# ubc-vision/quadraturefields

Measured on AMD Instinct MI355X. Metric: rays/sec at 800x800 Lego (mesh-quadrature render: ray/mesh intersection + hash-grid/MLP field + compositing), higher is better.
Workload: dtype f32; 1 GPU; Lego 800x800 (configs[1]), 1xMI355X per frame, fp32 hash-grid + tiny-MLP HIP kernels; rays_per_frame=640000, max_hits=25, triangles=983040, log2_hashmap_size=19, up_sample=1, bvh_fallback_frames=0, overflow_repaired_frames=8, reorigin_rule_redone_frames=0, camera_mismatch_frames=0, frames_in_flight=1

## Files before the change

### quadraturefields_amd/csrc/raster.hip

```cpp
#include <type_traits>

#include "exact_common.h"

#pragma clang fp contract(off)

namespace {

struct RasterCam {
    float r00, r01, r02, r10, r11, r12, r20, r21, r22;
    float cx, cy, cz;
    float fx, fy, px0, py0;
    int w, h;
};

constexpr float kRasterGuard = 0.25f;

struct SlabArgs {
    float t_lo, t_hi;
    int stop_at;
    uint64_t *keys;
    const float4 *ray_rec;
};

struct TriSetup {
    int x0, x1, y0, y1;
    bool use_edges;
    float ea[3], eb[3], ec[3];
};

__device__ __forceinline__ bool tri_setup(const float4 a, const float4 b, const float4 c, const RasterCam &cam, TriSetup &s)
{
    float minx = INFINITY, maxx = -INFINITY, miny = INFINITY, maxy = -INFINITY;
    int behind = 0;
    const float4 vs[3] = {a, b, c};
    float sxs[3], sys[3];
#pragma unroll
    for (int k = 0; k < 3; ++k) {
        const float dx = vs[k].x - cam.cx, dy = vs[k].y - cam.cy, dz = vs[k].z - cam.cz;
        const float xc = cam.r00 * dx + cam.r10 * dy + cam.r20 * dz;
        const float yc = cam.r01 * dx + cam.r11 * dy + cam.r21 * dz;
        const float zc = cam.r02 * dx + cam.r12 * dy + cam.r22 * dz;
        const float zv = -zc;
        if (!(zv > 1e-6f)) { ++behind; sxs[k] = sys[k] = 0.0f; continue; }
        const float sx = cam.fx * (xc / zv) + cam.px0;
        const float sy = -cam.fy * (yc / zv) + cam.py0;
        sxs[k] = sx; sys[k] = sy;
        minx = fminf(minx, sx); maxx = fmaxf(maxx, sx);
        miny = fminf(miny, sy); maxy = fmaxf(maxy, sy);
    }
    if (behind == 3) return false;
    s.use_edges = false;
    if (behind > 0) {
        s.x0 = 0; s.y0 = 0; s.x1 = cam.w - 1; s.y1 = cam.h - 1;
    } else {
        s.x0 = (int)fmaxf(floorf(minx - kRasterGuard), 0.0f);
        s.y0 = (int)fmaxf(floorf(miny - kRasterGuard), 0.0f);
        s.x1 = (int)fminf(ceilf(maxx + kRasterGuard), (float)(cam.w - 1));
        s.y1 = (int)fminf(ceilf(maxy + kRasterGuard), (float)(cam.h - 1));
        if (!(maxx + kRasterGuard >= 0.0f) || !(maxy + kRasterGuard >= 0.0f) ||
            !(minx - kRasterGuard <= (float)(cam.w - 1)) || !(miny - kRasterGuard <= (float)(cam.h - 1)))
            return false;
        const float area2 = (sxs[1] - sxs[0]) * (sys[2] - sys[0]) - (sys[1] - sys[0]) * (sxs[2] - sxs[0]);
        if (fabsf(area2) > 1e-2f) {
            s.use_edges = true;
            const float sgn = area2 > 0.0f ? 1.0f : -1.0f;
#pragma unroll
            for (int k = 0; k < 3; ++k) {
                const int k1 = (k + 1) % 3;
                const float ex = sxs[k1] - sxs[k], ey = sys[k1] - sys[k];
                s.ea[k] = -sgn * ey;
                s.eb[k] = sgn * ex;
                s.ec[k] = -(s.ea[k] * sxs[k] + s.eb[k] * sys[k]) + (kRasterGuard + 0.05f) * (fabsf(ex) + fabsf(ey)) + 1e-3f;
            }
        }
    }
    return true;
}

constexpr int kBinStage = 256;
constexpr int kBinIdBits = 26;
struct BinStage { int n; int tile[kBinStage]; uint2 rec[kBinStage]; };
struct TileBins {
    int32_t *cursor;
    uint2 *bins;
    int cap;
    BinStage *stage;
};

__device__ __forceinline__ void bin_records(const TileBins &tb, int tile, uint2 rec)
{
    const int lane = (int)__lane_id();
    for (;;) {
        const int t0 = __builtin_amdgcn_readfirstlane(tile);
        const unsigned long long m = __ballot(tile == t0);
        if (tile == t0) {
            const int rank = __popcll(m & ((1ull << lane) - 1ull));
            int base = 0;
            if (rank == 0) base = atomicAdd(&tb.cursor[t0], __popcll(m));
            base = __shfl(base, __ffsll((long long)m) - 1, 64);
            if (base + rank < tb.cap) tb.bins[(int64_t)t0 * tb.cap + base + rank] = rec;
            break;
        }
    }
}

template <int kRasterLanes, bool kWide, bool kSlab = false, bool kBins = false>
__device__ __forceinline__ void raster_triangle(const float4 *__restrict__ tris, int64_t tri_i, int sub, const RasterCam &cam,
                                                const float *__restrict__ rays_o, const float *__restrict__ rays_d,
                                                int max_hits, int32_t *__restrict__ hit_tri, float *__restrict__ hit_t,
                                                int32_t *__restrict__ hit_count, int32_t *__restrict__ overflow,
                                                const bool cam_origin, const SlabArgs slab = SlabArgs(),
                                                const TileBins bins = TileBins())
{
    const float4 a = tris[tri_i * 3 + 0], b = tris[tri_i * 3 + 1], c = tris[tri_i * 3 + 2];
    const int id = __float_as_int(a.w);
    TriSetup ts;
    if (!tri_setup(a, b, c, cam, ts)) return;
    const int x0 = ts.x0, x1 = ts.x1, y0 = ts.y0, y1 = ts.y1;
    const bool use_edges = ts.use_edges;
    const float *ea = ts.ea, *eb = ts.eb, *ec = ts.ec;
    const int bw = x1 - x0 + 1;
    const int total = bw * (y1 - y0 + 1);
    int px = x0 + sub % bw, py = y0 + sub / bw;
    for (int q = sub; q < total; q += kRasterLanes) {
        const int cx_ = px, cy_ = py;
        px += kRasterLanes;
        while (px > x1) { px -= bw; ++py; }
        if (use_edges) {
            const float fx_ = (float)cx_, fy_ = (float)cy_;
            if (ea[0] * fx_ + eb[0] * fy_ + ec[0] < 0.0f || ea[1] * fx_ + eb[1] * fy_ + ec[1] < 0.0f ||
                ea[2] * fx_ + eb[2] * fy_ + ec[2] < 0.0f)
                continue;
        }
        const int64_t ray = (int64_t)cy_ * cam.w + cx_;
        float dx, dy, dz;
        if (kSlab && slab.ray_rec) {
            const float4 rr = slab.ray_rec[ray];
            if (__float_as_int(rr.w) >= slab.stop_at) continue;
            dx = rr.x; dy = rr.y; dz = rr.z;
        } else {
            dx = rays_d[ray * 3]; dy = rays_d[ray * 3 + 1]; dz = rays_d[ray * 3 + 2];
        }
        float ox = cam.cx, oy = cam.cy, oz = cam.cz;
        if (!cam_origin) { ox = rays_o[ray * 3]; oy = rays_o[ray * 3 + 1]; oz = rays_o[ray * 3 + 2]; }
        asm volatile("" : "+v"(ox), "+v"(oy), "+v"(oz), "+v"(dx), "+v"(dy), "+v"(dz));
        float t;
        if (!mt_hit(a, b, c, ox, oy, oz, dx, dy, dz, &t)) continue;
        if (kSlab) {
            if (!(t >= slab.t_lo && t < slab.t_hi)) continue;
            const int slot = atomicAdd(&hit_count[ray], 1);
            if (slot < max_hits) slab.keys[(int64_t)slot * ((int64_t)cam.w * cam.h) + ray] = hit_key(t, id);
            else atomicAdd(overflow, 1);
            continue;
        }
        if (kBins) {
            const int tile = (cy_ >> 3) * ((cam.w + 7) >> 3) + (cx_ >> 3);
            const uint2 rec = make_uint2(__float_as_uint(t), ((uint32_t)id << 6) | (uint32_t)((cy_ & 7) * 8 + (cx_ & 7)));
            const int at = atomicAdd(&bins.stage->n, 1);
            if (at < kBinStage) { bins.stage->tile[at] = tile; bins.stage->rec[at] = rec; }
            else bin_records(bins, tile, rec);
            continue;
        }
        const int slot = atomicAdd(&hit_count[ray], 1);
        if (slot < max_hits) {
            const int64_t at = kWide ? (int64_t)slot * ((int64_t)cam.w * cam.h) + ray : ray * max_hits + slot;
            hit_t[at] = t;
            if (hit_tri) hit_tri[at] = id;
        } else {
            atomicAdd(overflow, 1);
        }
    }
}

template <int kRasterLanes, bool kWide>
__global__ __launch_bounds__(256) void raster_kernel(const float4 *__restrict__ tris, int64_t n_tri, RasterCam cam,
                                                     const float *__restrict__ rays_o, const float *__restrict__ rays_d,
                                                     int max_hits, int32_t *__restrict__ hit_tri, float *__restrict__ hit_t,
                                                     int32_t *__restrict__ hit_count, int32_t *__restrict__ overflow,
                                                     const int32_t *__restrict__ ray_flag)
{
    const int64_t gid = (int64_t)blockIdx.x * blockDim.x + threadIdx.x;
    const int64_t tri_i = gid / kRasterLanes;
    const int sub = (int)(gid % kRasterLanes);
    if (tri_i >= n_tri) return;
    if (ray_flag && *ray_flag) return;
    const bool cam_origin = ray_flag != nullptr;
    raster_triangle<kRasterLanes, kWide>(tris, tri_i, sub, cam, rays_o, rays_d, max_hits, hit_tri, hit_t, hit_count, overflow,
                                         cam_origin);
}

template <int kRasterLanes>
__global__ __launch_bounds__(256) void raster_bins_kernel(const float4 *__restrict__ tris, int64_t n_tri, RasterCam cam,
                                                          const float *__restrict__ rays_o, const float *__restrict__ rays_d,
                                                          int max_hits, int32_t *__restrict__ tile_cursor,
                                                          uint2 *__restrict__ bin_records_out,
                                                          const int32_t *__restrict__ ray_flag)
{
    __shared__ BinStage s_stage[4];
    const int64_t gid = (int64_t)blockIdx.x * blockDim.x + threadIdx.x;
    const int64_t tri_i = gid / kRasterLanes;
    const int sub = (int)(gid % kRasterLanes);
    if (ray_flag && *ray_flag) return;
    const bool cam_origin = ray_flag != nullptr;
    const int lane = (int)(threadIdx.x & 63);
    TileBins tb;
    tb.cursor = tile_cursor;
    tb.bins = bin_records_out;
    tb.cap = 64 * max_hits;
    tb.stage = &s_stage[threadIdx.x >> 6];
    if (lane == 0) tb.stage->n = 0;
    __builtin_amdgcn_fence(__ATOMIC_ACQ_REL, "workgroup");
    __builtin_amdgcn_wave_barrier();
    if (tri_i < n_tri)
        raster_triangle<kRasterLanes, false, false, true>(tris, tri_i, sub, cam, rays_o, rays_d, max_hits, nullptr, nullptr,
                                                          nullptr, nullptr, cam_origin, SlabArgs(), tb);
    __builtin_amdgcn_fence(__ATOMIC_ACQ_REL, "workgroup");
    __builtin_amdgcn_wave_barrier();
    const int n = tb.stage->n < kBinStage ? tb.stage->n : kBinStage;
    for (int i = lane; i < n; i += 64) bin_records(tb, tb.stage->tile[i], tb.stage->rec[i]);
}

__global__ __launch_bounds__(64) void tile_count_kernel(const int32_t *__restrict__ tile_cursor, const uint2 *__restrict__ bins,
                                                        int max_hits, int w, int h, int tiles_x,
                                                        int32_t *__restrict__ hit_count, int32_t *__restrict__ overflow,
                                                        uint64_t *__restrict__ tile_mask)
{
    __shared__ int s_cnt[64];
    const int tile = blockIdx.x, lane = threadIdx.x;
    const int cap = 64 * max_hits;
    const int cursor = tile_cursor[tile];
    const int n = cursor < cap ? cursor : cap;
    const int px = (tile % tiles_x) * 8 + (lane & 7), py = (tile / tiles_x) * 8 + (lane >> 3);
    const bool inside = px < w && py < h;
    int c = 0;
    if (n > 0) {
        s_cnt[lane] = 0;
        __syncthreads();
        const uint2 *run = bins + (int64_t)tile * cap;
        for (int i = lane; i < n; i += 64) atomicAdd(&s_cnt[run[i].y & 63u], 1);
        __syncthreads();
        c = s_cnt[lane];
    }
    int over = c > max_hits ? c - max_hits : 0;
    if (cursor > cap) {
        c = c > max_hits ? c : max_hits + 1;
        over = lane == 0 ? cursor - cap : 0;
    }
    if (inside) hit_count[(int64_t)py * w + px] = c;
    const unsigned long long mask = __ballot(inside && c > max_hits);
    if (mask) {
#pragma unroll
        for (int off = 32; off > 0; off >>= 1) over += __shfl_xor(over, off, 64);
        if (lane == 0) atomicAdd(overflow, over);
    }
    if (lane == 0) tile_mask[tile] = mask;
}

constexpr float kRayPixelTol = 0.02f;
constexpr float kRayUnitTol = 1e-4f;

__device__ __forceinline__ void camera_rays_check(const uint32_t *__restrict__ o_bits, const float *__restrict__ rays_d,
                                                  int64_t n_rays, const RasterCam &cam, int32_t *__restrict__ flag,
                                                  int64_t first, int64_t stride)
{
    const uint32_t c0 = __float_as_uint(cam.cx), c1 = __float_as_uint(cam.cy), c2 = __float_as_uint(cam.cz);
    bool bad = false;
    for (int64_t r = first; r < n_rays; r += stride) {
        const uint32_t o0 = o_bits[r * 3], o1 = o_bits[r * 3 + 1], o2 = o_bits[r * 3 + 2];
        const float dx = rays_d[r * 3], dy = rays_d[r * 3 + 1], dz = rays_d[r * 3 + 2];
        bad = bad || o0 != c0 || o1 != c1 || o2 != c2;
        const float xc = cam.r00 * dx + cam.r10 * dy + cam.r20 * dz;
        const float yc = cam.r01 * dx + cam.r11 * dy + cam.r21 * dz;
        const float zv = -(cam.r02 * dx + cam.r12 * dy + cam.r22 * dz);
        const float sx = cam.fx * (xc / zv) + cam.px0, sy = -cam.fy * (yc / zv) + cam.py0;
        const float px = (float)(int)(r % cam.w), py = (float)(int)(r / cam.w);
        bad = bad || !(zv > 0.0f) || !(fabsf(sx - px) <= kRayPixelTol) || !(fabsf(sy - py) <= kRayPixelTol) ||
              !(fabsf(dx * dx + dy * dy + dz * dz - 1.0f) <= kRayUnitTol);
    }
    if (bad) *flag = 1;
}

__global__ void camera_rays_check_kernel(const uint32_t *__restrict__ o_bits, const float *__restrict__ rays_d, int64_t n_rays,
                                         RasterCam cam, int32_t *__restrict__ flag)
{
    camera_rays_check(o_bits, rays_d, n_rays, cam, flag, (int64_t)blockIdx.x * blockDim.x + threadIdx.x,
                      (int64_t)gridDim.x * blockDim.x);
}

constexpr int kCullChunk = 64;

__global__ __launch_bounds__(256) void chunk_boxes_kernel(const float4 *__restrict__ tris, int64_t n_tri, int n_chunks,
                                                          float4 *__restrict__ boxes)
{
    const int chunk = (int)(((int64_t)blockIdx.x * blockDim.x + threadIdx.x) >> 6), lane = threadIdx.x & 63;
    if (chunk >= n_chunks) return;
    const int64_t t = (int64_t)chunk * kCullChunk + lane;
    float lo[3] = {INFINITY, INFINITY, INFINITY}, hi[3] = {-INFINITY, -INFINITY, -INFINITY};
    if (t < n_tri) {
#pragma unroll
        for (int k = 0; k < 3; ++k) {
            const float4 v = tris[t * 3 + k];
            lo[0] = fminf(lo[0], v.x); lo[1] = fminf(lo[1], v.y); lo[2] = fminf(lo[2], v.z);
            hi[0] = fmaxf(hi[0], v.x); hi[1] = fmaxf(hi[1], v.y); hi[2] = fmaxf(hi[2], v.z);
        }
    }
#pragma unroll
    for (int off = 32; off > 0; off >>= 1) {
#pragma unroll
        for (int k = 0; k < 3; ++k) {
            lo[k] = fminf(lo[k], __shfl_xor(lo[k], off, 64));
            hi[k] = fmaxf(hi[k], __shfl_xor(hi[k], off, 64));
        }
    }
    if (lane == 0) {
        boxes[chunk * 2 + 0] = make_float4(lo[0], lo[1], lo[2], 0.0f);
        boxes[chunk * 2 + 1] = make_float4(hi[0], hi[1], hi[2], 0.0f);
    }
}

__global__ void cull_chunks_kernel(const float4 *__restrict__ boxes, int n_chunks, RasterCam cam, int32_t *__restrict__ visible,
                                   int32_t *__restrict__ counters, int parity, const uint32_t *__restrict__ o_bits,
                                   const float *__restrict__ rays_d, int64_t n_rays, int32_t *__restrict__ ray_flag)
{
    const int chunk = blockIdx.x * blockDim.x + threadIdx.x;
    if (chunk == 0) counters[parity ^ 1] = 0;
    if (ray_flag) camera_rays_check(o_bits, rays_d, n_rays, cam, ray_flag, chunk, (int64_t)gridDim.x * blockDim.x);
    if (chunk >= n_chunks) return;
    const float4 lo = boxes[chunk * 2], hi = boxes[chunk * 2 + 1];
    if (!(lo.x <= hi.x)) return;
    float minx = INFINITY, maxx = -INFINITY, miny = INFINITY, maxy = -INFINITY;
    bool keep = false;
#pragma unroll
    for (int k = 0; k < 8; ++k) {
        const float dx = ((k & 1) ? hi.x : lo.x) - cam.cx, dy = ((k & 2) ? hi.y : lo.y) - cam.cy, dz = ((k & 4) ? hi.z : lo.z) - cam.cz;
        const float xc = cam.r00 * dx + cam.r10 * dy + cam.r20 * dz;
        const float yc = cam.r01 * dx + cam.r11 * dy + cam.r21 * dz;
        const float zc = cam.r02 * dx + cam.r12 * dy + cam.r22 * dz;
        const float zv = -zc;
        if (!(zv > 1e-4f)) { keep = true; continue; }
        const float sx = cam.fx * (xc / zv) + cam.px0, sy = -cam.fy * (yc / zv) + cam.py0;
        minx = fminf(minx, sx); maxx = fmaxf(maxx, sx);
        miny = fminf(miny, sy); maxy = fmaxf(maxy, sy);
    }
    const float g = kRasterGuard + 1.0f;
    if (!keep)
        keep = (maxx + g >= 0.0f) && (maxy + g >= 0.0f) && (minx - g <= (float)(cam.w - 1)) && (miny - g <= (float)(cam.h - 1));
    if (keep) visible[atomicAdd(&counters[parity], 1)] = chunk;
}

template <int kRasterLanes, bool kWide>
__global__ __launch_bounds__(256) void raster_culled_kernel(const float4 *__restrict__ tris, int64_t n_tri, RasterCam cam,
                                                            const float *__restrict__ rays_o, const float *__restrict__ rays_d,
                                                            int max_hits, int32_t *__restrict__ hit_tri, float *__restrict__ hit_t,
                                                            int32_t *__restrict__ hit_count, int32_t *__restrict__ overflow,
                                                            const int32_t *__restrict__ visible, const int32_t *__restrict__ n_visible,
                                                            const int32_t *__restrict__ ray_flag)
{
    if (ray_flag && *ray_flag) return;
    const bool cam_origin = ray_flag != nullptr;
    constexpr int kTrisPerBlock = 256 / kRasterLanes;
    constexpr int kBlocksPerChunk = kCullChunk / kTrisPerBlock;
    const int n_items = *n_visible * kBlocksPerChunk;
    const int sub = threadIdx.x % kRasterLanes;
    for (int item = blockIdx.x; item < n_items; item += gridDim.x) {
        const int chunk = visible[item / kBlocksPerChunk];
        const int64_t tri_i = (int64_t)chunk * kCullChunk + (item % kBlocksPerChunk) * kTrisPerBlock + threadIdx.x / kRasterLanes;
        if (tri_i < n_tri)
            raster_triangle<kRasterLanes, kWide>(tris, tri_i, sub, cam, rays_o, rays_d, max_hits, hit_tri, hit_t, hit_count, overflow,
                                                 cam_origin);
    }
}

constexpr int kMaxSlabs = 16;

struct SlabCtl {
    uint32_t dist_min_bits, dist_max_bits;
    int32_t n_visible;
    int32_t slab_count[kMaxSlabs];
};

__device__ __forceinline__ void slab_range(const SlabCtl *ctl, int n_slabs, float *lo, float *width)
{
    const float dmin = __uint_as_float(ctl->dist_min_bits) * 0.999f, dmax = __uint_as_float(ctl->dist_max_bits) * 1.001f;
    *lo = dmin;
    *width = fmaxf(dmax - dmin, 1e-12f) / (float)n_slabs;
}

__device__ __forceinline__ void slab_edges(const SlabCtl *ctl, int n_slabs, int j, float *t_lo, float *t_hi)
{
#pragma clang fp contract(off)
    float lo, w;
    slab_range(ctl, n_slabs, &lo, &w);
    *t_lo = j == 0 ? -INFINITY : lo + (float)j * w;
    *t_hi = j == n_slabs - 1 ? INFINITY : lo + (float)(j + 1) * w;
}

__global__ void slab_init_kernel(SlabCtl *ctl)
{
    ctl->dist_min_bits = 0x7f800000u;
    ctl->dist_max_bits = 0u;
    ctl->n_visible = 0;
    for (int j = 0; j < kMaxSlabs; ++j) ctl->slab_count[j] = 0;
}

__global__ void slab_cull_kernel(const float4 *__restrict__ boxes, int n_chunks, RasterCam cam, int32_t *__restrict__ visible,
                                 float2 *__restrict__ range, SlabCtl *ctl)
{
    const int chunk = blockIdx.x * blockDim.x + threadIdx.x;
    if (chunk >= n_chunks) return;
    const float4 lo = boxes[chunk * 2], hi = boxes[chunk * 2 + 1];
    if (!(lo.x <= hi.x)) return;
    float minx = INFINITY, maxx = -INFINITY, miny = INFINITY, maxy = -INFINITY;
    bool keep = false;
#pragma unroll
    for (int k = 0; k < 8; ++k) {
        const float dx = ((k & 1) ? hi.x : lo.x) - cam.cx, dy = ((k & 2) ? hi.y : lo.y) - cam.cy, dz = ((k & 4) ? hi.z : lo.z) - cam.cz;
        const float xc = cam.r00 * dx + cam.r10 * dy + cam.r20 * dz;
        const float yc = cam.r01 * dx + cam.r11 * dy + cam.r21 * dz;
        const float zc = cam.r02 * dx + cam.r12 * dy + cam.r22 * dz;
        const float zv = -zc;
        if (!(zv > 1e-4f)) { keep = true; continue; }
        const float sx = cam.fx * (xc / zv) + cam.px0, sy = -cam.fy * (yc / zv) + cam.py0;
        minx = fminf(minx, sx); maxx = fmaxf(maxx, sx);
        miny = fminf(miny, sy); maxy = fmaxf(maxy, sy);
    }
    const float g = kRasterGuard + 1.0f;
    if (!keep)
        keep = (maxx + g >= 0.0f) && (maxy + g >= 0.0f) && (minx - g <= (float)(cam.w - 1)) && (miny - g <= (float)(cam.h - 1));
    if (!keep) return;
    const float nx = fmaxf(fmaxf(lo.x - cam.cx, cam.cx - hi.x), 0.0f), ny = fmaxf(fmaxf(lo.y - cam.cy, cam.cy - hi.y), 0.0f);
    const float nz = fmaxf(fmaxf(lo.z - cam.cz, cam.cz - hi.z), 0.0f);
    const float fx = fmaxf(fabsf(lo.x - cam.cx), fabsf(hi.x - cam.cx)), fy = fmaxf(fabsf(lo.y - cam.cy), fabsf(hi.y - cam.cy));
    const float fz = fmaxf(fabsf(lo.z - cam.cz), fabsf(hi.z - cam.cz));
    const float dmin = sqrtf(nx * nx + ny * ny + nz * nz) * 0.9999f, dmax = sqrtf(fx * fx + fy * fy + fz * fz) * 1.0001f + 1e-30f;
    visible[atomicAdd(&ctl->n_visible, 1)] = chunk;
    range[chunk] = make_float2(dmin, dmax);
    atomicMin(&ctl->dist_min_bits, __float_as_uint(dmin));
    atomicMax(&ctl->dist_max_bits, __float_as_uint(dmax));
}

__global__ __launch_bounds__(256) void slab_assign_kernel(const int32_t *__restrict__ visible, const float2 *__restrict__ range,
                                                          SlabCtl *ctl, int n_slabs, int n_chunks, int32_t *__restrict__ lists)
{
    __shared__ int s_cnt[kMaxSlabs], s_base[kMaxSlabs];
    if (threadIdx.x < kMaxSlabs) s_cnt[threadIdx.x] = 0;
    __syncthreads();
    const int e = blockIdx.x * blockDim.x + threadIdx.x;
    int chunk = -1, j0 = 0, j1 = -1;
    if (e < ctl->n_visible) {
        chunk = visible[e];
        const float2 r = range[chunk];
        const float dlo = r.x * 0.999f, dhi = r.y * 1.001f;
        j0 = n_slabs;
        for (int j = 0; j < n_slabs; ++j) {
            float t_lo, t_hi;
            slab_edges(ctl, n_slabs, j, &t_lo, &t_hi);
            if (t_hi > dlo && t_lo <= dhi) { j0 = j < j0 ? j : j0; j1 = j; }
        }
        for (int j = j0; j <= j1; ++j) atomicAdd(&s_cnt[j], 1);
    }
    __syncthreads();
    if (threadIdx.x < n_slabs) s_base[threadIdx.x] = s_cnt[threadIdx.x] ? atomicAdd(&ctl->slab_count[threadIdx.x], s_cnt[threadIdx.x]) : 0;
    __syncthreads();
    for (int j = j0; j <= j1; ++j) lists[(int64_t)j * n_chunks + atomicAdd(&s_base[j], 1)] = chunk;
}

__global__ void slab_ray_records_kernel(const float *__restrict__ rays_d, const int32_t *__restrict__ hit_count, int64_t n,
                                        float4 *__restrict__ rec)
{
    for (int64_t i = (int64_t)blockIdx.x * blockDim.x + threadIdx.x; i < n; i += (int64_t)gridDim.x * blockDim.x)
        rec[i] = make_float4(rays_d[i * 3], rays_d[i * 3 + 1], rays_d[i * 3 + 2], __int_as_float(hit_count[i]));
}

template <int kRasterLanes>
__global__ __launch_bounds__(256) void raster_slab_kernel(const float4 *__restrict__ tris, int64_t n_tri, RasterCam cam,
                                                          const float *__restrict__ rays_o, const float *__restrict__ rays_d,
                                                          int capacity, uint64_t *__restrict__ keys, int32_t *__restrict__ hit_count,
                                                          int32_t *__restrict__ overflow, const int32_t *__restrict__ list,
                                                          const SlabCtl *__restrict__ ctl, int slab_j, int n_slabs, int stop_at,
                                                          const float4 *__restrict__ ray_rec,
                                                          const int32_t *__restrict__ ray_flag)
{
    if (ray_flag && *ray_flag) return;
    const bool cam_origin = ray_flag != nullptr;
    constexpr int kTrisPerBlock = 256 / kRasterLanes;
    constexpr int kBlocksPerChunk = kCullChunk / kTrisPerBlock;
    const int n_items = ctl->slab_count[slab_j] * kBlocksPerChunk;
    SlabArgs sa;
    slab_edges(ctl, n_slabs, slab_j, &sa.t_lo, &sa.t_hi);
    sa.stop_at = stop_at;
    sa.keys = keys;
    sa.ray_rec = ray_rec;
    const int sub = threadIdx.x % kRasterLanes;
    for (int item = blockIdx.x; item < n_items; item += gridDim.x) {
        const int chunk = list[item / kBlocksPerChunk];
        const int64_t tri_i = (int64_t)chunk * kCullChunk + (item % kBlocksPerChunk) * kTrisPerBlock + threadIdx.x / kRasterLanes;
        if (tri_i < n_tri)
            raster_triangle<kRasterLanes, true, true>(tris, tri_i, sub, cam, rays_o, rays_d, capacity, nullptr, nullptr,
                                                      hit_count, overflow, cam_origin, sa);
    }
}

constexpr int kSelectBlock = 64;
constexpr int kSelectHeadroom = 8;
__host__ __device__ inline int select_capacity(int max_hits, int wide, float min_sep)
{
    const int cap = min_sep > 0.0f ? max_hits + kSelectHeadroom : max_hits;
    return cap < wide ? cap : wide;
}
__device__ __forceinline__ void write_row_from_keys(const uint64_t *lk, int count, float *row_t, int32_t *row_i)
{
    int i = 0;
    for (; i + 4 <= count; i += 4) {
        f32x4u t4;
        i32x4u i4;
#pragma unroll
        for (int e = 0; e < 4; ++e) {
            const uint64_t k = lk[(i + e) * kSelectBlock];
            t4[e] = key_t(k);
            i4[e] = key_id(k);
        }
        *reinterpret_cast<f32x4u *>(row_t + i) = t4;
        *reinterpret_cast<i32x4u *>(row_i + i) = i4;
    }
    for (; i < count; ++i) {
        const uint64_t k = lk[i * kSelectBlock];
        row_t[i] = key_t(k);
        row_i[i] = key_id(k);
    }
}

template <bool kKeys>
__global__ __launch_bounds__(kSelectBlock) void select_nearest_kernel(int64_t n_rays, int wide, int max_hits, float min_sep,
                                                                      const int32_t *__restrict__ wide_tri,
                                                                      const float *__restrict__ wide_t,
                                                                      const uint64_t *__restrict__ wide_key,
                                                                      int32_t *__restrict__ hit_tri, float *__restrict__ hit_t,
                                                                      int32_t *__restrict__ hit_count)
{
    extern __shared__ __attribute__((aligned(8))) unsigned char select_lds[];
    const int cap = select_capacity(max_hits, wide, min_sep);
    uint64_t *lk = reinterpret_cast<uint64_t *>(select_lds) + threadIdx.x;
    const int64_t r = (int64_t)blockIdx.x * kSelectBlock + threadIdx.x;
    if (r >= n_rays) return;
    const int cnt = hit_count[r];
    if (cnt > wide) return;
    float *row_t = hit_t + r * max_hits;
    int32_t *row_i = hit_tri + r * max_hits;
    if (cnt <= max_hits) {
        constexpr int kCopy = 8;
        for (int i0 = 0; i0 < cnt; i0 += kCopy) {
            float tb[kCopy];
            int ib[kCopy];
#pragma unroll
            for (int u = 0; u < kCopy; ++u) {
                const int i = i0 + u < cnt ? i0 + u : cnt - 1;
                if (kKeys) {
                    const uint64_t k = wide_key[(int64_t)i * n_rays + r];
                    tb[u] = key_t(k);
                    ib[u] = key_id(k);
                } else {
                    tb[u] = wide_t[(int64_t)i * n_rays + r];
                    ib[u] = wide_tri[(int64_t)i * n_rays + r];
                }
            }
#pragma unroll
            for (int q = 0; q < kCopy / 4; ++q) {
                if (i0 + 4 * q + 4 <= cnt) {
                    *reinterpret_cast<f32x4u *>(row_t + i0 + 4 * q) = (f32x4u){tb[4 * q], tb[4 * q + 1], tb[4 * q + 2], tb[4 * q + 3]};
                    *reinterpret_cast<i32x4u *>(row_i + i0 + 4 * q) = (i32x4u){ib[4 * q], ib[4 * q + 1], ib[4 * q + 2], ib[4 * q + 3]};
                } else {
#pragma unroll
                    for (int e = 0; e < 4; ++e)
                        if (i0 + 4 * q + e < cnt) { row_t[i0 + 4 * q + e] = tb[4 * q + e]; row_i[i0 + 4 * q + e] = ib[4 * q + e]; }
                }
            }
        }
        return;
    }
    const int held = cnt < cap ? cnt : cap;
    constexpr int kBatch = 8;
    int n = 0;
    uint64_t max_key = 0;
    for (int i0 = 0; i0 < cnt; i0 += kBatch) {
        uint64_t kb[kBatch];
#pragma unroll
        for (int u = 0; u < kBatch; ++u) {
            const int i = i0 + u < cnt ? i0 + u : cnt - 1;
            if (kKeys) kb[u] = wide_key[(int64_t)i * n_rays + r];
            else kb[u] = hit_key(wide_t[(int64_t)i * n_rays + r], wide_tri[(int64_t)i * n_rays + r]);
        }
#pragma unroll
        for (int u = 0; u < kBatch; ++u) {
            if (i0 + u >= cnt) break;
            const uint64_t key = kb[u];
            int m;
            if (n < held) {
                m = n;
                ++n;
            } else {
                if (!(key < max_key)) continue;
                m = n - 1;
            }
            int lo = 0, hi = m;
            while (lo < hi) {
                const int mid = (lo + hi) >> 1;
                if (lk[mid * kSelectBlock] < key) lo = mid + 1;
                else hi = mid;
            }
            int j = m - 1;
            for (; j - 3 >= lo; j -= 4) {
                const uint64_t a0 = lk[j * kSelectBlock], a1 = lk[(j - 1) * kSelectBlock], a2 = lk[(j - 2) * kSelectBlock],
                               a3 = lk[(j - 3) * kSelectBlock];
                lk[(j + 1) * kSelectBlock] = a0;
                lk[j * kSelectBlock] = a1;
                lk[(j - 1) * kSelectBlock] = a2;
                lk[(j - 2) * kSelectBlock] = a3;
            }
            for (; j >= lo; --j) lk[(j + 1) * kSelectBlock] = lk[j * kSelectBlock];
            lk[lo * kSelectBlock] = key;
            max_key = lk[(n - 1) * kSelectBlock];
        }
    }
    if (min_sep <= 0.0f) {
        write_row_from_keys(lk, max_hits, row_t, row_i);
        hit_count[r] = max_hits;
        return;
    }
    float last_t = key_t(lk[0]);
    int kept = 1;
    for (int i = 1; i < held && kept < max_hits; ++i) {
        const uint64_t k = lk[i * kSelectBlock];
        const float t = key_t(k);
        if (!(t > last_t + min_sep)) continue;
        last_t = t;
        lk[kept * kSelectBlock] = k;
        ++kept;
    }
    if (kept < max_hits && cnt > held) return;
    write_row_from_keys(lk, kept, row_t, row_i);
    hit_count[r] = kept;
}

constexpr int kFilterRays = 128;
__global__ __launch_bounds__(kFilterRays) void filter_hits_kernel(int64_t n_rays, int max_hits, float min_sep,
                                                                  int32_t *__restrict__ hit_tri, float *__restrict__ hit_t,
                                                                  int32_t *__restrict__ hit_count)
{
    extern __shared__ __attribute__((aligned(16))) unsigned char filter_smem[];
    const int K = max_hits, Kp = max_hits | 1;
    float *s_t = reinterpret_cast<float *>(filter_smem);
    int32_t *s_tri = reinterpret_cast<int32_t *>(s_t + kFilterRays * Kp);
    const int tid = threadIdx.x;
    const int64_t ray0 = (int64_t)blockIdx.x * kFilterRays;
    const int nr = (int)((n_rays - ray0) < kFilterRays ? (n_rays - ray0) : kFilterRays);
    for (int i = tid; i < nr * K; i += kFilterRays) {
        const int r = i / K, k = i - r * K;
        s_t[r * Kp + k] = hit_t[ray0 * K + i];
        s_tri[r * Kp + k] = hit_tri[ray0 * K + i];
    }
    __syncthreads();
    if (tid < nr) {
        int cnt = hit_count[ray0 + tid];
        if (cnt > K) cnt = K;
        float *row_t = s_t + tid * Kp;
        int32_t *row_i = s_tri + tid * Kp;
        if (K <= 32) {
            if (cnt > 1) sort_row_32<true>(row_t, row_i, cnt);
        } else {
            for (int i = 1; i < cnt; ++i) {
                const float t = row_t[i];
                const int id = row_i[i];
                int j = i - 1;
                while (j >= 0 && hit_less(t, id, row_t[j], row_i[j])) { row_t[j + 1] = row_t[j]; row_i[j + 1] = row_i[j]; --j; }
                row_t[j + 1] = t;
                row_i[j + 1] = id;
            }
        }
        if (min_sep > 0.0f && cnt > 1) {
            int kept = 1;
            float last_t = row_t[0];
            for (int i = 1; i < cnt; ++i) {
                const float t = row_t[i];
                if (t > last_t + min_sep) { row_t[kept] = t; row_i[kept] = row_i[i]; ++kept; last_t = t; }
            }
            cnt = kept;
        }
        for (int i = cnt; i < K; ++i) { row_t[i] = INFINITY; row_i[i] = -1; }
        hit_count[ray0 + tid] = cnt;
    }
    __syncthreads();
    for (int i = tid; i < nr * K; i += kFilterRays) {
        const int r = i / K, k = i - r * K;
        hit_t[ray0 * K + i] = s_t[r * Kp + k];
        hit_tri[ray0 * K + i] = s_tri[r * Kp + k];
    }
}

}

static int filter_launch(int64_t n_rays, int32_t max_hits, float min_sep, int32_t *hit_tri, float *hit_t,
                         int32_t *hit_count, hipStream_t st)
{
    const int Kp = max_hits | 1;
    const size_t lds = (size_t)kFilterRays * Kp * 8;
    const int64_t blocks = qf_div_up(n_rays, kFilterRays);
    if (blocks > 0x7fffffff) return QF_ERR_UNSUPPORTED;
    hipLaunchKernelGGL(filter_hits_kernel, dim3((unsigned)blocks), dim3(kFilterRays), lds, st, n_rays, (int)max_hits, min_sep,
                       hit_tri, hit_t, hit_count);
    QF_LAUNCH_CHECK();
    return QF_OK;
}

extern "C" int qf_filter_hits(const qf_bvh *bvh, int64_t n_rays, int32_t max_hits, int32_t *hit_tri, float *hit_t,
                              int32_t *hit_count, void *stream)
{
    if (!bvh || n_rays < 0 || max_hits < 1 || max_hits > kMaxHits) return QF_ERR_INVALID_ARGUMENT;
    if (n_rays == 0 || !(bvh->min_sep > 0.0f)) return QF_OK;
    if (!hit_tri || !hit_t || !hit_count) return QF_ERR_INVALID_ARGUMENT;
    return filter_launch(n_rays, max_hits, bvh->min_sep, hit_tri, hit_t, hit_count, qf_stream(stream));
}

static RasterCam make_raster_cam(const qf_camera *cam)
{
    RasterCam rc;
    const float *m = cam->c2w;
    rc.r00 = m[0]; rc.r01 = m[1]; rc.r02 = m[2]; rc.cx = m[3];
    rc.r10 = m[4]; rc.r11 = m[5]; rc.r12 = m[6]; rc.cy = m[7];
    rc.r20 = m[8]; rc.r21 = m[9]; rc.r22 = m[10]; rc.cz = m[11];
    rc.fx = cam->fx; rc.fy = cam->fy;
    rc.px0 = cam->cx - 0.5f;
    rc.py0 = cam->cy - 0.5f;
    rc.w = cam->width; rc.h = cam->height;
    return rc;
}

static int ensure_chunk_boxes(qf_bvh *bvh, hipStream_t st)
{
    const int64_t n_chunks = qf_div_up(bvh->n_tri, kCullChunk);
    if (n_chunks > 0x3fffffff) return QF_ERR_UNSUPPORTED;
    if (!bvh->d_chunk_box) {
        QF_HIP_TRY(hipMalloc((void **)&bvh->d_chunk_box, (size_t)n_chunks * 2 * sizeof(float4)));
        QF_HIP_TRY(hipMalloc((void **)&bvh->d_visible, (size_t)(n_chunks + 2) * sizeof(int32_t)));
        QF_HIP_TRY(hipMemsetAsync(bvh->d_visible, 0, 2 * sizeof(int32_t), st));
        bvh->chunk_dirty = true;
        bvh->cull_parity = 0;
    }
    if (bvh->chunk_dirty) {
        hipLaunchKernelGGL(chunk_boxes_kernel, dim3((unsigned)qf_div_up(n_chunks * 64, 256)), dim3(256), 0, st,
                           reinterpret_cast<const float4 *>(bvh->d_tris), bvh->n_tri, (int)n_chunks,
                           reinterpret_cast<float4 *>(bvh->d_chunk_box));
        QF_LAUNCH_CHECK();
        bvh->chunk_dirty = false;
    }
    return QF_OK;
}

static int raster_zero(int64_t n_rays, int32_t *hit_count, int32_t *overflow, int32_t *origin_flag, hipStream_t st)
{
    int64_t words = n_rays;
    bool ovf_done = false, flag_done = origin_flag == nullptr;
    if (overflow == hit_count + words) { ++words; ovf_done = true; }
    if (ovf_done && origin_flag == hit_count + words) { ++words; flag_done = true; }
    QF_HIP_TRY(hipMemsetAsync(hit_count, 0, (size_t)words * sizeof(int32_t), st));
    if (!ovf_done) QF_HIP_TRY(hipMemsetAsync(overflow, 0, sizeof(int32_t), st));
    if (!flag_done) QF_HIP_TRY(hipMemsetAsync(origin_flag, 0, sizeof(int32_t), st));
    return QF_OK;
}

static int raster_lanes(int64_t n_rays, int64_t n_tri)
{
    const int64_t pixels_per_tri = n_rays / n_tri;
    return pixels_per_tri > 64 ? 16 : (pixels_per_tri > 8 ? 8 : 4);
}

template <typename F>
static void with_lanes(int lanes, F &&f)
{
    switch (lanes) {
    case 16: f(std::integral_constant<int, 16>()); break;
    case 8: f(std::integral_constant<int, 8>()); break;
    default: f(std::integral_constant<int, 4>()); break;
    }
}

static unsigned chunk_grid(int64_t n_chunks, int lanes)
{
    const int64_t items = n_chunks * (kCullChunk * lanes / 256);
    const int64_t cap = (int64_t)qf_cu_count_cached() * 8;
    return (unsigned)(items < cap ? items : cap);
}

static void camera_check_launch(const RasterCam &rc, const float *rays_o, const float *rays_d, int64_t n_rays,
                                int32_t *origin_flag, hipStream_t st)
{
    if (origin_flag)
        hipLaunchKernelGGL(camera_rays_check_kernel, dim3(qf_grid_1d(n_rays, 256)), dim3(256), 0, st,
                           reinterpret_cast<const uint32_t *>(rays_o), rays_d, n_rays, rc, origin_flag);
}

static int raster_launch(qf_bvh *bvh, const qf_camera *cam, const float *rays_o, const float *rays_d, int64_t n_rays,
                         int capacity, bool wide, int32_t *hit_tri, float *hit_t, int32_t *hit_count, int32_t *overflow,
                         int32_t *origin_flag, bool cull, hipStream_t st, bool skip_ids = false)
{
    if (skip_ids) hit_tri = nullptr;
    const int rc_zero = raster_zero(n_rays, hit_count, overflow, origin_flag, st);
    if (rc_zero != QF_OK) return rc_zero;
    if (bvh->n_tri == 0) return QF_OK;
    const RasterCam rc = make_raster_cam(cam);
    const float4 *tris4 = reinterpret_cast<const float4 *>(bvh->d_tris);
    const int lanes = raster_lanes(n_rays, bvh->n_tri);
    const int64_t blocks = qf_div_up(bvh->n_tri * lanes, 256);
    if (blocks > 0x7fffffff) return QF_ERR_UNSUPPORTED;
    if (cull) {
        const int64_t n_chunks = qf_div_up(bvh->n_tri, kCullChunk);
        const int rc_boxes = ensure_chunk_boxes(bvh, st);
        if (rc_boxes != QF_OK) return rc_boxes;
        float4 *boxes = reinterpret_cast<float4 *>(bvh->d_chunk_box);
        int32_t *counters = bvh->d_visible, *visible = bvh->d_visible + 2;
        const int parity = bvh->cull_parity;
        bvh->cull_parity ^= 1;
        bvh->cull_last = parity;
        hipLaunchKernelGGL(cull_chunks_kernel, dim3((unsigned)qf_div_up(n_chunks, 256)), dim3(256), 0, st, boxes,
                           (int)n_chunks, rc, visible, counters, parity, reinterpret_cast<const uint32_t *>(rays_o), rays_d,
                           n_rays, origin_flag);
        QF_LAUNCH_CHECK();
        with_lanes(lanes, [&](auto L) {
            auto *kernel = wide ? raster_culled_kernel<decltype(L)::value, true> : raster_culled_kernel<decltype(L)::value, false>;
            hipLaunchKernelGGL(kernel, dim3(chunk_grid(n_chunks, lanes)), dim3(256), 0, st, tris4, bvh->n_tri, rc, rays_o, rays_d,
                               capacity, hit_tri, hit_t, hit_count, overflow, visible, counters + parity, origin_flag);
        });
    } else {
        camera_check_launch(rc, rays_o, rays_d, n_rays, origin_flag, st);
        QF_LAUNCH_CHECK();
        with_lanes(lanes, [&](auto L) {
            auto *kernel = wide ? raster_kernel<decltype(L)::value, true> : raster_kernel<decltype(L)::value, false>;
            hipLaunchKernelGGL(kernel, dim3((unsigned)blocks), dim3(256), 0, st, tris4, bvh->n_tri, rc, rays_o, rays_d, capacity,
                               hit_tri, hit_t, hit_count, overflow, origin_flag);
        });
    }
    QF_LAUNCH_CHECK();
    return QF_OK;
}

static bool raster_args_ok(const qf_bvh *bvh, const qf_camera *cam, int64_t n_rays, int32_t max_hits)
{
    if (!bvh || !cam || n_rays < 0 || max_hits < 1 || max_hits > kMaxHits) return false;
    if (cam->width < 1 || cam->height < 1 || (int64_t)cam->width * cam->height != n_rays) return false;
    return cam->fx > 0.0f && cam->fy > 0.0f;
}

extern "C" int qf_raster_intersect(qf_bvh *bvh, const qf_camera *cam, const float *rays_o, const float *rays_d,
                                   int64_t n_rays, int32_t max_hits, int32_t *hit_tri, float *hit_t, int32_t *hit_count,
                                   int32_t *overflow, int32_t sort_lists, int32_t cull_chunks, int32_t *origin_flag,
                                   void *stream)
{
    if (!raster_args_ok(bvh, cam, n_rays, max_hits)) return QF_ERR_INVALID_ARGUMENT;
    if (!rays_o || !rays_d || !hit_tri || !hit_t || !hit_count || !overflow) return QF_ERR_INVALID_ARGUMENT;
    if (sort_lists < 0 || sort_lists > 2) return QF_ERR_INVALID_ARGUMENT;
    hipStream_t st = qf_stream(stream);
    const int rc = raster_launch(bvh, cam, rays_o, rays_d, n_rays, (int)max_hits, false, hit_tri, hit_t, hit_count, overflow,
                                 origin_flag, cull_chunks != 0, st, sort_lists == 2);
    if (rc != QF_OK) return rc;
    if (sort_lists == 1 && n_rays > 0) return filter_launch(n_rays, max_hits, bvh->min_sep, hit_tri, hit_t, hit_count, st);
    return QF_OK;
}

extern "C" int64_t qf_hit_bins_bytes(int32_t width, int32_t height, int32_t max_hits)
{
    if (width < 1 || height < 1 || max_hits < 1 || max_hits > kMaxHits) return -1;
    return (int64_t)((width + 7) / 8) * ((height + 7) / 8) * 64 * max_hits * (int64_t)sizeof(uint2);
}

extern "C" int qf_raster_intersect_tiles(qf_bvh *bvh, const qf_camera *cam, const float *rays_o, const float *rays_d,
                                         int64_t n_rays, int32_t max_hits, int32_t *tile_cursor, uint64_t *tile_mask,
                                         void *bins, int64_t bins_bytes, int32_t *hit_count, int32_t *overflow,
                                         int32_t *origin_flag, void *stream)
{
    if (!raster_args_ok(bvh, cam, n_rays, max_hits)) return QF_ERR_INVALID_ARGUMENT;
    if (!rays_o || !rays_d || !tile_cursor || !tile_mask || !bins || !hit_count || !overflow) return QF_ERR_INVALID_ARGUMENT;
    if (bins_bytes < qf_hit_bins_bytes(cam->width, cam->height, max_hits)) return QF_ERR_INVALID_ARGUMENT;
    if (reinterpret_cast<uintptr_t>(bins) % sizeof(uint2) || reinterpret_cast<uintptr_t>(tile_mask) % sizeof(uint64_t))
        return QF_ERR_INVALID_ARGUMENT;
    if (bvh->n_tri >= (1 << kBinIdBits)) return QF_ERR_UNSUPPORTED;
    hipStream_t st = qf_stream(stream);
    const int tiles_x = (cam->width + 7) / 8, n_tiles = tiles_x * ((cam->height + 7) / 8);
    QF_HIP_TRY(hipMemsetAsync(tile_cursor, 0, (size_t)n_tiles * sizeof(int32_t), st));
    if (origin_flag == overflow + 1) {
        QF_HIP_TRY(hipMemsetAsync(overflow, 0, 2 * sizeof(int32_t), st));
    } else {
        QF_HIP_TRY(hipMemsetAsync(overflow, 0, sizeof(int32_t), st));
        if (origin_flag) QF_HIP_TRY(hipMemsetAsync(origin_flag, 0, sizeof(int32_t), st));
    }
    const RasterCam rc = make_raster_cam(cam);
    uint2 *records = reinterpret_cast<uint2 *>(bins);
    if (bvh->n_tri > 0) {
        const int lanes = raster_lanes(n_rays, bvh->n_tri);
        const int64_t blocks = qf_div_up(bvh->n_tri * lanes, 256);
        if (blocks > 0x7fffffff) return QF_ERR_UNSUPPORTED;
        camera_check_launch(rc, rays_o, rays_d, n_rays, origin_flag, st);
        QF_LAUNCH_CHECK();
        with_lanes(lanes, [&](auto L) {
            hipLaunchKernelGGL(raster_bins_kernel<decltype(L)::value>, dim3((unsigned)blocks), dim3(256), 0, st,
                               reinterpret_cast<const float4 *>(bvh->d_tris), bvh->n_tri, rc, rays_o, rays_d, (int)max_hits,
                               tile_cursor, records, origin_flag);
        });
    }
    hipLaunchKernelGGL(tile_count_kernel, dim3((unsigned)n_tiles), dim3(64), 0, st, tile_cursor, records, (int)max_hits,
                       rc.w, rc.h, tiles_x, hit_count, overflow, tile_mask);
    QF_LAUNCH_CHECK();
    return QF_OK;
}

extern "C" int qf_raster_intersect_wide(qf_bvh *bvh, const qf_camera *cam, const float *rays_o, const float *rays_d,
                                        int64_t n_rays, int32_t max_hits, int32_t wide_hits, int32_t *wide_tri,
                                        float *wide_t, int32_t *hit_tri, float *hit_t, int32_t *hit_count,
                                        int32_t *overflow, int32_t cull_chunks, int32_t *origin_flag, void *stream)
{
    if (!raster_args_ok(bvh, cam, n_rays, max_hits)) return QF_ERR_INVALID_ARGUMENT;
    if (wide_hits < max_hits || wide_hits > 4096) return QF_ERR_INVALID_ARGUMENT;
    if (!rays_o || !rays_d || !wide_tri || !wide_t || !hit_tri || !hit_t || !hit_count || !overflow)
        return QF_ERR_INVALID_ARGUMENT;
    hipStream_t st = qf_stream(stream);
    const int rc = raster_launch(bvh, cam, rays_o, rays_d, n_rays, (int)wide_hits, true, wide_tri, wide_t, hit_count, overflow,
                                 origin_flag, cull_chunks != 0, st);
    if (rc != QF_OK) return rc;
    if (n_rays == 0) return QF_OK;
    const size_t lds = (size_t)select_capacity(max_hits, wide_hits, bvh->min_sep) * kSelectBlock * 2 * sizeof(float);
    hipLaunchKernelGGL(select_nearest_kernel<false>, dim3((unsigned)qf_div_up(n_rays, kSelectBlock)), dim3(kSelectBlock), lds, st,
                       n_rays, (int)wide_hits, (int)max_hits, bvh->min_sep, wide_tri, wide_t, (const uint64_t *)nullptr, hit_tri,
                       hit_t, hit_count);
    QF_LAUNCH_CHECK();
    return QF_OK;
}

extern "C" int qf_raster_intersect_slabs(qf_bvh *bvh, const qf_camera *cam, const float *rays_o, const float *rays_d,
                                         int64_t n_rays, int32_t max_hits, int32_t wide_hits, int32_t n_slabs,
                                         uint64_t *wide_keys, int32_t *hit_tri, float *hit_t, int32_t *hit_count,
                                         int32_t *overflow, int32_t *origin_flag, void *stream)
{
    if (!raster_args_ok(bvh, cam, n_rays, max_hits)) return QF_ERR_INVALID_ARGUMENT;
    if (n_slabs < 2 || n_slabs > kMaxSlabs) return QF_ERR_INVALID_ARGUMENT;
    const int sel_cap = select_capacity(max_hits, wide_hits, bvh->min_sep);
    if (wide_hits <= sel_cap + 1 || wide_hits > 4096) return QF_ERR_INVALID_ARGUMENT;
    if (!rays_o || !rays_d || !wide_keys || !hit_tri || !hit_t || !hit_count || !overflow) return QF_ERR_INVALID_ARGUMENT;
    hipStream_t st = qf_stream(stream);
    const int rc_zero = raster_zero(n_rays, hit_count, overflow, origin_flag, st);
    if (rc_zero != QF_OK) return rc_zero;
    if (n_rays == 0 || bvh->n_tri == 0) return QF_OK;
    const int rc_boxes = ensure_chunk_boxes(bvh, st);
    if (rc_boxes != QF_OK) return rc_boxes;
    const int64_t n_chunks = qf_div_up(bvh->n_tri, kCullChunk);
    if (!bvh->d_slab_range) {
        QF_HIP_TRY(hipMalloc((void **)&bvh->d_slab_range, (size_t)n_chunks * sizeof(float2)));
        QF_HIP_TRY(hipMalloc((void **)&bvh->d_slab_lists, (size_t)n_chunks * kMaxSlabs * sizeof(int32_t)));
        QF_HIP_TRY(hipMalloc((void **)&bvh->d_slab_ctl, sizeof(SlabCtl)));
    }
    const RasterCam rc = make_raster_cam(cam);
    const float4 *tris4 = reinterpret_cast<const float4 *>(bvh->d_tris);
    const float4 *boxes = reinterpret_cast<const float4 *>(bvh->d_chunk_box);
    int32_t *visible = bvh->d_visible + 2;
    bvh->cull_last = -1;
    float2 *range = reinterpret_cast<float2 *>(bvh->d_slab_range);
    SlabCtl *ctl = reinterpret_cast<SlabCtl *>(bvh->d_slab_ctl);
    camera_check_launch(rc, rays_o, rays_d, n_rays, origin_flag, st);
    hipLaunchKernelGGL(slab_init_kernel, dim3(1), dim3(1), 0, st, ctl);
    hipLaunchKernelGGL(slab_cull_kernel, dim3((unsigned)qf_div_up(n_chunks, 256)), dim3(256), 0, st, boxes, (int)n_chunks, rc,
                       visible, range, ctl);
    hipLaunchKernelGGL(slab_assign_kernel, dim3((unsigned)qf_div_up(n_chunks, 256)), dim3(256), 0, st, visible, range, ctl,
                       (int)n_slabs, (int)n_chunks, bvh->d_slab_lists);
    QF_LAUNCH_CHECK();
    const int lanes = raster_lanes(n_rays, bvh->n_tri);
    const unsigned grid = chunk_grid(n_chunks, lanes);
    const int stop_at = sel_cap + 1;
    if (bvh->slab_snapshot_rays < n_rays) {
        const int64_t grown = bvh->slab_snapshot_rays * 2 > n_rays ? bvh->slab_snapshot_rays * 2 : n_rays;
        if (bvh->d_slab_snapshot) (void)hipFree(bvh->d_slab_snapshot);
        bvh->d_slab_snapshot = nullptr;
        bvh->slab_snapshot_rays = 0;
        QF_HIP_TRY(hipMalloc((void **)&bvh->d_slab_snapshot, (size_t)grown * sizeof(float4)));
        bvh->slab_snapshot_rays = grown;
    }
    float4 *snapshot = reinterpret_cast<float4 *>(bvh->d_slab_snapshot);
    for (int j = 0; j < n_slabs; ++j) {
        if (j > 0) {
            hipLaunchKernelGGL(slab_ray_records_kernel, dim3(qf_grid_1d(n_rays, 256)), dim3(256), 0, st, rays_d, hit_count,
                               n_rays, snapshot);
            QF_LAUNCH_CHECK();
        }
        const int32_t *list = bvh->d_slab_lists + (int64_t)j * n_chunks;
        with_lanes(lanes, [&](auto L) {
            hipLaunchKernelGGL(raster_slab_kernel<decltype(L)::value>, dim3(grid), dim3(256), 0, st, tris4, bvh->n_tri, rc, rays_o,
                               rays_d, (int)wide_hits, wide_keys, hit_count, overflow, list, ctl, j, (int)n_slabs, stop_at,
                               j == 0 ? (const float4 *)nullptr : snapshot, origin_flag);
        });
    }
    QF_LAUNCH_CHECK();
    const size_t lds = (size_t)sel_cap * kSelectBlock * 2 * sizeof(float);
    hipLaunchKernelGGL(select_nearest_kernel<true>, dim3((unsigned)qf_div_up(n_rays, kSelectBlock)), dim3(kSelectBlock), lds, st,
                       n_rays, (int)wide_hits, (int)max_hits, bvh->min_sep, (const int32_t *)nullptr, (const float *)nullptr,
                       wide_keys, hit_tri, hit_t, hit_count);
    QF_LAUNCH_CHECK();
    return QF_OK;
}

extern "C" int64_t qf_bvh_copy_visible_chunks(const qf_bvh *bvh, int32_t *chunks_host, int64_t capacity, void *stream)
{
    if (!bvh || capacity < 0 || (capacity > 0 && !chunks_host)) return QF_ERR_INVALID_ARGUMENT;
    if (!bvh->d_visible || bvh->cull_last < 0) return QF_ERR_INVALID_ARGUMENT;
    QF_HIP_TRY(hipStreamSynchronize(qf_stream(stream)));
    int32_t n = 0;
    QF_HIP_TRY(hipMemcpy(&n, bvh->d_visible + bvh->cull_last, sizeof(int32_t), hipMemcpyDeviceToHost));
    const int64_t n_chunks = qf_div_up(bvh->n_tri, kCullChunk);
    if (n < 0 || n > n_chunks) return QF_ERR_HIP;
    const int64_t take = n < capacity ? n : capacity;
    if (take > 0) QF_HIP_TRY(hipMemcpy(chunks_host, bvh->d_visible + 2, (size_t)take * sizeof(int32_t), hipMemcpyDeviceToHost));
    return n;
}
```

Measured before the change: 407.4 million rays/s.

## Add wave-compacted triangle rasterization kernel with LDS pixel queues for binning

Adds a new binning kernel where each 64-lane wave owns 64 triangles. A prefix scan over per-triangle bounding-box work splits the boxes into row pieces, and edge tests then push surviving pixels into an LDS ring queue. Exact Möller–Trumbore tests run in full 64-lane rounds, and hits are staged in a second ring before being binned. The aim is to remove the lane divergence and load imbalance of the fixed lanes-per-triangle kernel, in exchange for heavy LDS use, wave-level syncs and different record ordering.

Result: no change. 405.1 million rays/s (-0.6%).

```diff
diff --git a/quadraturefields_amd/csrc/raster.hip b/quadraturefields_amd/csrc/raster.hip
--- a/quadraturefields_amd/csrc/raster.hip
+++ b/quadraturefields_amd/csrc/raster.hip
@@ -218,6 +218,160 @@
     __builtin_amdgcn_wave_barrier();
     const int n = tb.stage->n < kBinStage ? tb.stage->n : kBinStage;
     for (int i = lane; i < n; i += 64) bin_records(tb, tb.stage->tile[i], tb.stage->rec[i]);
+}
+
+constexpr int64_t kCompactMaxRays = 1 << 25;
+constexpr int kCompactPiece = 64;
+constexpr int kCompactRing = 128;
+struct CompactWave {
+    float4 va[64], vb[64], vc[64];
+    int4 box[64];
+    float4 e0[64], e1[64], e2[64];
+    int4 start4[16];
+    int qx[kCompactRing], qy[kCompactRing], qs[kCompactRing];
+    int stile[kCompactRing];
+    uint2 srec[kCompactRing];
+};
+
+__device__ __forceinline__ int lanes_below(unsigned long long m)
+{
+    return (int)__builtin_amdgcn_mbcnt_hi((unsigned)(m >> 32), __builtin_amdgcn_mbcnt_lo((unsigned)m, 0u));
+}
+
+__device__ __forceinline__ void wave_lds_sync()
+{
+    __builtin_amdgcn_fence(__ATOMIC_ACQ_REL, "workgroup");
+    __builtin_amdgcn_wave_barrier();
+}
+
+__global__ __launch_bounds__(64) void raster_bins_compact_kernel(const float4 *__restrict__ tris, int64_t n_tri, RasterCam cam,
+                                                                 const float *__restrict__ rays_o, const float *__restrict__ rays_d,
+                                                                 int max_hits, int32_t *__restrict__ tile_cursor,
+                                                                 uint2 *__restrict__ bin_records_out,
+                                                                 const int32_t *__restrict__ ray_flag)
+{
+    __shared__ CompactWave s;
+    if (ray_flag && *ray_flag) return;
+    const bool cam_origin = ray_flag != nullptr;
+    const int lane = (int)threadIdx.x;
+    TileBins tb;
+    tb.cursor = tile_cursor;
+    tb.bins = bin_records_out;
+    tb.cap = 64 * max_hits;
+    tb.stage = nullptr;
+
+    const int64_t tri_i = (int64_t)blockIdx.x * 64 + lane;
+    TriSetup ts = {};
+    int n_box = 0;
+    if (tri_i < n_tri) {
+        const float4 a = tris[tri_i * 3 + 0], b = tris[tri_i * 3 + 1], c = tris[tri_i * 3 + 2];
+        s.va[lane] = a; s.vb[lane] = b; s.vc[lane] = c;
+        if (tri_setup(a, b, c, cam, ts)) n_box = ((ts.x1 - ts.x0 + kCompactPiece) / kCompactPiece) * (ts.y1 - ts.y0 + 1);
+        else ts = TriSetup{};
+    }
+    int incl = n_box;
+#pragma unroll
+    for (int off = 1; off < 64; off <<= 1) {
+        const int up = __shfl_up(incl, off, 64);
+        if (lane >= off) incl += up;
+    }
+    const int start = incl - n_box;
+    const int total = __builtin_amdgcn_readlane(incl, 63);
+    s.box[lane] = make_int4(ts.x0, ts.y0, ts.x1 - ts.x0 + 1, start);
+    s.e0[lane] = make_float4(ts.ea[0], ts.eb[0], ts.ec[0], __int_as_float(ts.use_edges ? 1 : 0));
+    s.e1[lane] = make_float4(ts.ea[1], ts.eb[1], ts.ec[1], 0.0f);
+    s.e2[lane] = make_float4(ts.ea[2], ts.eb[2], ts.ec[2], 0.0f);
+    reinterpret_cast<int *>(s.start4)[lane] = start;
+    const int p1 = __builtin_amdgcn_readlane(start, 8), p2 = __builtin_amdgcn_readlane(start, 16),
+              p3 = __builtin_amdgcn_readlane(start, 24), p4 = __builtin_amdgcn_readlane(start, 32),
+              p5 = __builtin_amdgcn_readlane(start, 40), p6 = __builtin_amdgcn_readlane(start, 48),
+              p7 = __builtin_amdgcn_readlane(start, 56);
+    const int tiles_x = (cam.w + 7) >> 3;
+    int q_head = 0, q_tail = 0, s_head = 0, s_tail = 0;
+
+    auto exact_round = [&](const int count) {
+        wave_lds_sync();
+        bool hit = false;
+        int tile = 0;
+        uint2 rec = make_uint2(0u, 0u);
+        if (lane < count) {
+            const int at = (q_head + lane) & (kCompactRing - 1);
+            const int cx_ = s.qx[at], cy_ = s.qy[at], slot = s.qs[at];
+            const float4 a = s.va[slot], b = s.vb[slot], c = s.vc[slot];
+            const int64_t ray = (int64_t)cy_ * cam.w + cx_;
+            float dx = rays_d[ray * 3], dy = rays_d[ray * 3 + 1], dz = rays_d[ray * 3 + 2];
+            float ox = cam.cx, oy = cam.cy, oz = cam.cz;
+            if (!cam_origin) { ox = rays_o[ray * 3]; oy = rays_o[ray * 3 + 1]; oz = rays_o[ray * 3 + 2]; }
+            asm volatile("" : "+v"(ox), "+v"(oy), "+v"(oz), "+v"(dx), "+v"(dy), "+v"(dz));
+            float t;
+            if (mt_hit(a, b, c, ox, oy, oz, dx, dy, dz, &t)) {
+                hit = true;
+                tile = (cy_ >> 3) * tiles_x + (cx_ >> 3);
+                rec = make_uint2(__float_as_uint(t),
+                                 ((uint32_t)__float_as_int(a.w) << 6) | (uint32_t)((cy_ & 7) * 8 + (cx_ & 7)));
+            }
+        }
+        q_head += count;
+        const unsigned long long hits = __ballot(hit);
+        if (hit) {
+            const int at = (s_tail + lanes_below(hits)) & (kCompactRing - 1);
+            s.stile[at] = tile;
+            s.srec[at] = rec;
+        }
+        s_tail += __popcll(hits);
+        if (s_tail - s_head >= 64) {
+            wave_lds_sync();
+            const int at = (s_head + lane) & (kCompactRing - 1);
+            bin_records(tb, s.stile[at], s.srec[at]);
+            s_head += 64;
+        }
+    };
+
+    wave_lds_sync();
+    for (int base = 0; base < total; base += 64) {
+        const int g = base + lane;
+        const bool valid = g < total;
+        const int c8 = (g >= p1) + (g >= p2) + (g >= p3) + (g >= p4) + (g >= p5) + (g >= p6) + (g >= p7);
+        const int4 lo = s.start4[2 * c8], hi = s.start4[2 * c8 + 1];
+        const int slot = 8 * c8 + (g >= lo.y) + (g >= lo.z) + (g >= lo.w) + (g >= hi.x) + (g >= hi.y) + (g >= hi.z) + (g >= hi.w);
+        const int4 box = s.box[slot];
+        const float4 e0 = s.e0[slot], e1 = s.e1[slot], e2 = s.e2[slot];
+        const int r = valid ? g - box.w : 0, bw = box.z;
+        int row = r, x_first = box.x, len = bw;
+        if (bw > kCompactPiece) {
+            const int per_row = (bw + kCompactPiece - 1) / kCompactPiece;
+            row = r / per_row;
+            const int off = (r - row * per_row) * kCompactPiece;
+            x_first += off;
+            len = bw - off < kCompactPiece ? bw - off : kCompactPiece;
+        }
+        if (!valid) len = 0;
+        const int cy_ = box.y + row;
+        const float fy_ = (float)cy_;
+        const float b0 = e0.y * fy_, b1 = e1.y * fy_, b2 = e2.y * fy_;
+        const bool use_edges = __float_as_int(e0.w) != 0;
+        for (int i = 0; i < kCompactPiece; ++i) {
+            const bool active = i < len;
+            if (!__any(active)) break;
+            const int cx_ = x_first + i;
+            const float fx_ = (float)cx_;
+            const bool outside = e0.x * fx_ + b0 + e0.z < 0.0f || e1.x * fx_ + b1 + e1.z < 0.0f || e2.x * fx_ + b2 + e2.z < 0.0f;
+            const bool keep = active && !(use_edges && outside);
+            const unsigned long long kept = __ballot(keep);
+            if (keep) {
+                const int at = (q_tail + lanes_below(kept)) & (kCompactRing - 1);
+                s.qx[at] = cx_; s.qy[at] = cy_; s.qs[at] = slot;
+            }
+            q_tail += __popcll(kept);
+            if (q_tail - q_head >= 64) exact_round(64);
+        }
+    }
+    if (q_tail > q_head) exact_round(q_tail - q_head);
+    wave_lds_sync();
+    if (lane < s_tail - s_head) {
+        const int at = (s_head + lane) & (kCompactRing - 1);
+        bin_records(tb, s.stile[at], s.srec[at]);
+    }
 }
 
 __global__ __launch_bounds__(64) void tile_count_kernel(const int32_t *__restrict__ tile_cursor, const uint2 *__restrict__ bins,
@@ -900,7 +1054,11 @@
         if (blocks > 0x7fffffff) return QF_ERR_UNSUPPORTED;
         camera_check_launch(rc, rays_o, rays_d, n_rays, origin_flag, st);
         QF_LAUNCH_CHECK();
-        with_lanes(lanes, [&](auto L) {
+        if (n_rays < kCompactMaxRays)
+            hipLaunchKernelGGL(raster_bins_compact_kernel, dim3((unsigned)qf_div_up(bvh->n_tri, 64)), dim3(64), 0, st,
+                               reinterpret_cast<const float4 *>(bvh->d_tris), bvh->n_tri, rc, rays_o, rays_d, (int)max_hits,
+                               tile_cursor, records, origin_flag);
+        else with_lanes(lanes, [&](auto L) {
             hipLaunchKernelGGL(raster_bins_kernel<decltype(L)::value>, dim3((unsigned)blocks), dim3(256), 0, st,
                                reinterpret_cast<const float4 *>(bvh->d_tris), bvh->n_tri, rc, rays_o, rays_d, (int)max_hits,
                                tile_cursor, records, origin_flag);
```
